# seung-lab/chunkflow

Hardware: AMD Instinct MI355X
Metric: output_voxels_per_sec (higher is better)
Workload: dtype f32; 1 GPU; config2-512cube-rsunet-affinity; batch_size=12, engine=rsunet

## Files before the change

chunkflow_amd/csrc/conv.hip:

```cpp
#include <hip/hip_runtime.h>

#include "cfx_internal.h"

namespace {

typedef float f32x4 __attribute__((ext_vector_type(4)));

constexpr int padc(int C) {
    return (C % 32 == 0 || C % 32 == 16) ? C + 4 : C;
}

template <int C, int K, int TZv, int TY, int TX, int TAPG, int NTHREADS>
__global__ __launch_bounds__(NTHREADS, 1) void k_conv3(
    const float* __restrict__ in,
    const float* __restrict__ wgt,
    const float* __restrict__ bias,
    const float* __restrict__ res,
    float* __restrict__ out,
    int N, int D, int H, int W, int do_elu) {
    constexpr int PC = padc(C);
    constexpr int SX = TX + 2;
    constexpr int SY = TY + 2;
    constexpr int SZ = TZv + 2;
    constexpr int KK = C / 4;
    constexpr int NT = (K + 15) / 16;
    constexpr int NW = NTHREADS / 64;
    constexpr int XT = TX / 16;
    constexpr int M_TILES = (TZv * TY * XT) / NW;
    static_assert((TZv * TY * XT) % NW == 0, "tiles must split evenly");

    __shared__ float slab[SZ * SY * SX * PC];
    __shared__ float wtile[TAPG * NT * C * 16];

    const int bx = blockIdx.x;
    const int by = blockIdx.y;
    const int bzn = blockIdx.z;
    const int zblocks = (D + TZv - 1) / TZv;
    const int n = bzn / zblocks;
    const int z0 = (bzn % zblocks) * TZv;
    const int y0 = by * TY;
    const int x0 = bx * TX;

    const int tid = threadIdx.x;
    const int wave = tid >> 6;
    const int lane = tid & 63;

    {
        const int c4n = C / 4;
        const int vox = SZ * SY * SX;
        const bool interior = z0 >= 1 && z0 + TZv + 1 <= D && y0 >= 1 &&
                              y0 + TY + 1 <= H && x0 >= 1 &&
                              x0 + TX + 1 <= W;
        const float* base =
            in + ((((long long)n * D + z0 - 1) * H + y0 - 1) * W + x0 - 1)
                 * C;
        if (interior) {
            for (int idx = tid; idx < vox * c4n; idx += NTHREADS) {
                const int c4 = idx % c4n;
                const int v = idx / c4n;
                const int sx = v % SX;
                const int sy = (v / SX) % SY;
                const int sz = v / (SX * SY);
                const f32x4 val = *reinterpret_cast<const f32x4*>(
                    base + (((long long)sz * H + sy) * W + sx) * C +
                    c4 * 4);
                *reinterpret_cast<f32x4*>(
                    &slab[((sz * SY + sy) * SX + sx) * PC + c4 * 4]) = val;
            }
        } else {
            for (int idx = tid; idx < vox * c4n; idx += NTHREADS) {
                const int c4 = idx % c4n;
                const int v = idx / c4n;
                const int sx = v % SX;
                const int sy = (v / SX) % SY;
                const int sz = v / (SX * SY);
                const int gz = z0 + sz - 1;
                const int gy = y0 + sy - 1;
                const int gx = x0 + sx - 1;
                const bool ok = gz >= 0 && gz < D && gy >= 0 && gy < H &&
                                gx >= 0 && gx < W;
                const int cz = ok ? gz : 0;
                const int cy = ok ? gy : 0;
                const int cx = ok ? gx : 0;
                f32x4 val = *reinterpret_cast<const f32x4*>(
                    in + ((((long long)n * D + cz) * H + cy) * W + cx) * C +
                    c4 * 4);
                if (!ok) val = {0.f, 0.f, 0.f, 0.f};
                *reinterpret_cast<f32x4*>(
                    &slab[((sz * SY + sy) * SX + sx) * PC + c4 * 4]) = val;
            }
        }
    }
    __syncthreads();

    int tmz[M_TILES], tmy[M_TILES], tmx[M_TILES];
#pragma unroll
    for (int m = 0; m < M_TILES; ++m) {
        const int g = wave * M_TILES + m;
        tmx[m] = (g % XT) * 16;
        tmy[m] = (g / XT) % TY;
        tmz[m] = g / (XT * TY);
    }

    f32x4 acc[M_TILES][NT];
#pragma unroll
    for (int m = 0; m < M_TILES; ++m)
#pragma unroll
        for (int t = 0; t < NT; ++t)
            acc[m][t] = {0.f, 0.f, 0.f, 0.f};

    const int a_row = lane & 15;
    const int a_k = lane >> 4;
    const int col16 = lane & 15;

    static_assert(27 % TAPG == 0, "TAPG must divide 27");
    for (int g = 0; g < 27 / TAPG; ++g) {
        for (int idx = tid; idx < TAPG * NT * C * 16;
             idx += NTHREADS) {
            const int j = idx & 15;
            const int c = (idx >> 4) % C;
            const int nt = (idx >> 4) / C % NT;
            const int tl = (idx >> 4) / C / NT;
            const int jg = nt * 16 + j;
            wtile[idx] = jg < K
                ? wgt[((long long)(g * TAPG + tl) * C + c) * K + jg]
                : 0.f;
        }
        __syncthreads();
#pragma unroll
        for (int tl = 0; tl < TAPG; ++tl) {
            const int tap = g * TAPG + tl;
            const int dz = tap / 9 - 1;
            const int dy = (tap / 3) % 3 - 1;
            const int dx = tap % 3 - 1;
            const float* arow[M_TILES];
#pragma unroll
            for (int m = 0; m < M_TILES; ++m) {
                arow[m] = &slab[(((1 + tmz[m] + dz) * SY +
                                  (1 + tmy[m] + dy)) * SX +
                                 (1 + tmx[m] + dx)) * PC + a_row * PC + a_k];
            }
            const float* wblk = &wtile[tl * NT * C * 16];
#pragma unroll
            for (int nt = 0; nt < NT; ++nt) {
#pragma unroll
                for (int kk = 0; kk < KK; ++kk) {
                    const float b =
                        wblk[(nt * C + kk * 4 + a_k) * 16 + col16];
#pragma unroll
                    for (int m = 0; m < M_TILES; ++m) {
                        const float a = arow[m][kk * 4];
                        acc[m][nt] = __builtin_amdgcn_mfma_f32_16x16x4f32(
                            a, b, acc[m][nt], 0, 0, 0);
                    }
                }
            }
        }
        __syncthreads();
    }

    const int col = lane & 15;
    const int rbase = (lane >> 4) * 4;
#pragma unroll
    for (int m = 0; m < M_TILES; ++m) {
        const int gz = z0 + tmz[m];
        const int gy = y0 + tmy[m];
        if (gz >= D || gy >= H) continue;
#pragma unroll
        for (int t = 0; t < NT; ++t) {
            const int j = t * 16 + col;
            if (j >= K) continue;
            const float bj = bias ? bias[j] : 0.f;
#pragma unroll
            for (int r = 0; r < 4; ++r) {
                const int gx = x0 + tmx[m] + rbase + r;
                if (gx >= W) continue;
                long long o =
                    ((((long long)n * D + gz) * H + gy) * W + gx) * K + j;
                float v = acc[m][t][r] + bj;
                if (res) v += res[o];
                if (do_elu) v = v > 0.f ? v : expm1f(v);
                out[o] = v;
            }
        }
    }
}

}

extern "C" int cfx_conv3_ndhwc(cfx_ctx* ctx, const float* in,
                               const float* wgt, const float* bias,
                               const float* residual, float* out, int N,
                               int D, int H, int W, int C, int K,
                               int do_elu) {
    if (C != K) {
        g_err = "cfx_conv3_ndhwc: only C == K widths are instantiated";
        return -1;
    }
#define CFX_CONV_CASE(CW, TZV, TYV, TXV, TAPGV, NTH)                         \
    case CW: {                                                               \
        const int zb = (D + TZV - 1) / TZV;                                  \
        dim3 grid((W + TXV - 1) / TXV, (H + TYV - 1) / TYV,                  \
                  (unsigned)(N * zb));                                       \
        hipEvent_t e0;                                                       \
        if (prof_begin(ctx, &e0)) return -1;                                 \
        hipLaunchKernelGGL((k_conv3<CW, CW, TZV, TYV, TXV, TAPGV, NTH>),     \
                           grid, dim3(NTH), 0, ctx->stream, in, wgt, bias,   \
                           residual, out, N, D, H, W, do_elu);               \
        CFX_CHECK(hipGetLastError());                                        \
        double flops = 2.0 * 27.0 * CW * CW * (double)N * D * H * W;         \
        if (prof_end(ctx, e0, CFX_K_CONV, flops)) return -1;                 \
        break;                                                               \
    }
    switch (C) {
        CFX_CONV_CASE(28, 1, 8, 32, 3, 512)
        CFX_CONV_CASE(36, 1, 8, 32, 1, 512)
        CFX_CONV_CASE(48, 1, 4, 32, 1, 512)
        CFX_CONV_CASE(64, 2, 2, 16, 1, 256)
        default:
            g_err = "cfx_conv3_ndhwc: unsupported channel width";
            return -1;
    }
#undef CFX_CONV_CASE
    return 0;
}

namespace {

template <int C, int K, int TY, int TAPG>
__global__ __launch_bounds__(512, 1) void k_conv3_w32(
    const float* __restrict__ in, const float* __restrict__ wgt,
    const float* __restrict__ bias, const float* __restrict__ res,
    float* __restrict__ out, int N, int D, int H, int W, int do_elu) {
    constexpr int TX = 32;
    constexpr int SX = TX + 2;
    constexpr int SY = TY + 2;
    constexpr int SZ = 3;
    constexpr int KK = C / 2;
    static_assert(K <= 32 && C % 2 == 0, "");

    __shared__ float slab[SZ * SY * C * SX];
    __shared__ float wtile[TAPG * C * 32];

    const int zblocks = D;
    const int n = blockIdx.z / zblocks;
    const int z0 = blockIdx.z % zblocks;
    const int y0 = blockIdx.y * TY;
    const int x0 = blockIdx.x * TX;
    const int tid = threadIdx.x;
    const int wave = tid >> 6;
    const int lane = tid & 63;

    {
        const int c4n = C / 4;
        const bool interior = z0 >= 1 && z0 + 2 <= D && y0 >= 1 &&
                              y0 + TY + 1 <= H && x0 >= 1 &&
                              x0 + TX + 1 <= W;
        for (int idx = tid; idx < SZ * SY * SX * c4n; idx += 512) {
            const int c4 = idx % c4n;
            const int v = idx / c4n;
            const int sx = v % SX;
            const int sy = (v / SX) % SY;
            const int sz = v / (SX * SY);
            const int gz = z0 + sz - 1;
            const int gy = y0 + sy - 1;
            const int gx = x0 + sx - 1;
            f32x4 val;
            if (interior) {
                val = *reinterpret_cast<const f32x4*>(
                    in + ((((long long)n * D + gz) * H + gy) * W + gx) * C +
                    c4 * 4);
            } else {
                const bool ok = gz >= 0 && gz < D && gy >= 0 && gy < H &&
                                gx >= 0 && gx < W;
                val = *reinterpret_cast<const f32x4*>(
                    in + ((((long long)n * D + (ok ? gz : 0)) * H +
                           (ok ? gy : 0)) * W + (ok ? gx : 0)) * C +
                    c4 * 4);
                if (!ok) val = {0.f, 0.f, 0.f, 0.f};
            }
            float* base = &slab[((sz * SY + sy) * C + c4 * 4) * SX + sx];
            base[0 * SX] = val.x;
            base[1 * SX] = val.y;
            base[2 * SX] = val.z;
            base[3 * SX] = val.w;
        }
    }
    __syncthreads();

    typedef float f32x16 __attribute__((ext_vector_type(16)));
    f32x16 acc = {};
    const int ax = lane & 31;
    const int ak = lane >> 5;

    static_assert(27 % TAPG == 0, "");
    for (int g = 0; g < 27 / TAPG; ++g) {
        for (int idx = tid; idx < TAPG * C * 32; idx += 512) {
            const int j = idx & 31;
            const int c = (idx >> 5) % C;
            const int tl = (idx >> 5) / C;
            wtile[idx] = j < K
                ? wgt[((long long)(g * TAPG + tl) * C + c) * K + j]
                : 0.f;
        }
        __syncthreads();
#pragma unroll
        for (int tl = 0; tl < TAPG; ++tl) {
            const int tap = g * TAPG + tl;
            const int dz = tap / 9 - 1;
            const int dy = (tap / 3) % 3 - 1;
            const int dx = tap % 3 - 1;
            const float* arow =
                &slab[((1 + dz) * SY + (1 + wave + dy)) * C * SX +
                      (1 + dx) + ax];
            const float* wrow = &wtile[tl * C * 32 + ax];
#pragma unroll
            for (int kk = 0; kk < KK; ++kk) {
                const float a = arow[(kk * 2 + ak) * SX];
                const float b = wrow[(kk * 2 + ak) * 32];
                acc = __builtin_amdgcn_mfma_f32_32x32x2f32(a, b, acc, 0, 0,
                                                           0);
            }
        }
        __syncthreads();
    }

    const int gz = z0;
    const int gy = y0 + wave;
    const int j = lane & 31;
    if (gy < H && j < K) {
        const float bj = bias ? bias[j] : 0.f;
#pragma unroll
        for (int r = 0; r < 16; ++r) {
            const int row = (r & 3) + 8 * (r >> 2) + 4 * (lane >> 5);
            const int gx = x0 + row;
            if (gx >= W) continue;
            long long o =
                ((((long long)n * D + gz) * H + gy) * W + gx) * K + j;
            float v = acc[r] + bj;
            if (res) v += res[o];
            if (do_elu) v = v > 0.f ? v : expm1f(v);
            out[o] = v;
        }
    }
}

}

extern "C" int cfx_conv3_ndhwc_w32(cfx_ctx* ctx, const float* in,
                                   const float* wgt, const float* bias,
                                   const float* residual, float* out, int N,
                                   int D, int H, int W, int C, int K,
                                   int do_elu) {
    if (C != 28 || K != 28) {
        g_err = "cfx_conv3_ndhwc_w32: only C == K == 28 instantiated";
        return -1;
    }
    dim3 grid((W + 31) / 32, (H + 7) / 8, (unsigned)(N * D));
    hipEvent_t e0;
    if (prof_begin(ctx, &e0)) return -1;
    hipLaunchKernelGGL((k_conv3_w32<28, 28, 8, 3>), grid, dim3(512), 0,
                       ctx->stream, in, wgt, bias, residual, out, N, D, H,
                       W, do_elu);
    CFX_CHECK(hipGetLastError());
    double flops = 2.0 * 27.0 * 28 * 28 * (double)N * D * H * W;
    if (prof_end(ctx, e0, CFX_K_CONV, flops)) return -1;
    return 0;
}

namespace {

template <int C, int K, int TY, int TX, int NTK>
__global__ __launch_bounds__(512, 1) void k_conv3_zring_pl(
    const float* __restrict__ in, const float* __restrict__ wgt,
    const float* __restrict__ bias, const float* __restrict__ res,
    float* __restrict__ out, int N, int D, int H, int W, int do_elu,
    int j0, int wvec) {
    constexpr int PC = padc(C);
    constexpr int SX = TX + 2;
    constexpr int SY = TY + 2;
    constexpr int KK = C / 4;
    constexpr int NT = NTK;
    constexpr int NW = 8;
    constexpr int XT = TX / 16;
    constexpr int M_TILES = (TY * XT) / NW;
    constexpr int C4N = C / 4;
    constexpr int LV = (SY * SX * C4N + 511) / 512;
    constexpr int WV4 = 27 * NT * C * 4;
    constexpr int WL = (WV4 + 511) / 512;
    static_assert((TY * XT) % NW == 0, "");

    __shared__ __attribute__((aligned(16))) float ring[3 * SY * SX * PC];
    __shared__ __attribute__((aligned(16))) float wall[27 * NT * C * 16];

    const int n = blockIdx.z;
    const int y0 = blockIdx.y * TY;
    const int x0 = blockIdx.x * TX;
    const int tid = threadIdx.x;
    const int wave = tid >> 6;
    const int lane = tid & 63;

    auto wall_load = [&](f32x4 (&wv)[WL], bool (&wk)[WL]) {
#pragma unroll
        for (int li = 0; li < WL; ++li) {
            const int idx = min(tid + li * 512, WV4 - 1);
            const int row = idx >> 2;
            const int c = row % C;
            const int nt = row / C % NT;
            const int tap = row / C / NT;
            const int jg = j0 + nt * 16 + (idx & 3) * 4;
            wk[li] = jg < K;
            wv[li] = *reinterpret_cast<const f32x4*>(
                wgt + ((long long)tap * C + c) * K + (jg < K ? jg : 0));
        }
    };
    auto wall_store = [&](const f32x4 (&wv)[WL], const bool (&wk)[WL]) {
#pragma unroll
        for (int li = 0; li < WL; ++li) {
            const int idx = tid + li * 512;
            if (idx >= WV4) break;
            *reinterpret_cast<f32x4*>(&wall[idx * 4]) =
                wk[li] ? wv[li] : f32x4{0.f, 0.f, 0.f, 0.f};
        }
    };
    if (!wvec) {
        for (int idx = tid; idx < 27 * NT * C * 16; idx += 512) {
            const int j = idx & 15;
            const int c = (idx >> 4) % C;
            const int nt = (idx >> 4) / C % NT;
            const int tap = (idx >> 4) / C / NT;
            const int jg = j0 + nt * 16 + j;
            wall[idx] =
                jg < K ? wgt[((long long)tap * C + c) * K + jg] : 0.f;
        }
    }

    const bool xy_interior = y0 >= 1 && y0 + TY + 1 <= H && x0 >= 1 &&
                             x0 + TX + 1 <= W;

    static_assert(SY * SX * C4N > 512 && SY * SX * C4N > (LV - 1) * 512, "");
    auto plane_idx = [&](int li) {
        const int idx = tid + li * 512;
        return idx < SY * SX * C4N ? idx : idx - 512;
    };
    auto plane_load = [&](int P, f32x4 (&vals)[LV], bool (&keep)[LV]) {
        const bool zin = P >= 0 && P < D;
        const bool interior = zin && xy_interior;
#pragma unroll
        for (int li = 0; li < LV; ++li) {
            const int idx = plane_idx(li);
            const int c4 = idx % C4N;
            const int v = idx / C4N;
            const int gy = y0 + v / SX - 1;
            const int gx = x0 + v % SX - 1;
            const bool ok = zin && (interior ||
                                    (gy >= 0 && gy < H && gx >= 0 &&
                                     gx < W));
            keep[li] = ok;
            vals[li] = *reinterpret_cast<const f32x4*>(
                in + ((((long long)n * D + (zin ? P : 0)) * H +
                       (ok ? gy : 0)) * W + (ok ? gx : 0)) * C + c4 * 4);
        }
    };
    auto plane_store = [&](int P, const f32x4 (&vals)[LV],
                           const bool (&keep)[LV]) {
        const int slot = ((P + 1) % 3 + 3) % 3;
#pragma unroll
        for (int li = 0; li < LV; ++li) {
            const int idx = plane_idx(li);
            const int c4 = idx % C4N;
            const int v = idx / C4N;
            *reinterpret_cast<f32x4*>(
                &ring[(slot * SY * SX + v) * PC + c4 * 4]) =
                keep[li] ? vals[li] : f32x4{0.f, 0.f, 0.f, 0.f};
        }
    };

    {
        f32x4 wv[WL];
        bool wk[WL];
        f32x4 v0[LV], v1[LV];
        bool k0[LV], k1[LV];
        if (wvec) wall_load(wv, wk);
        plane_load(-1, v0, k0);
        plane_load(0, v1, k1);
        if (wvec) wall_store(wv, wk);
        plane_store(-1, v0, k0);
        plane_store(0, v1, k1);
    }
    __syncthreads();

    int tmy[M_TILES], tmx[M_TILES];
#pragma unroll
    for (int m = 0; m < M_TILES; ++m) {
        const int g = wave * M_TILES + m;
        tmx[m] = (g % XT) * 16;
        tmy[m] = g / XT;
    }
    const int a_row = lane & 15;
    const int a_k = lane >> 4;
    const int col16 = lane & 15;
    const int colj = lane & 15;
    const int rbase = (lane >> 4) * 4;

    float bj[NT];
#pragma unroll
    for (int t = 0; t < NT; ++t)
        bj[t] = bias ? bias[min(j0 + t * 16 + colj, K - 1)] : 0.f;

    for (int z = 0; z < D; ++z) {
        f32x4 acc[M_TILES][NT];
        f32x4 acc2[M_TILES];
#pragma unroll
        for (int m = 0; m < M_TILES; ++m) {
            acc2[m] = {0.f, 0.f, 0.f, 0.f};
#pragma unroll
            for (int t = 0; t < NT; ++t)
                acc[m][t] = {0.f, 0.f, 0.f, 0.f};
        }

        auto compute_dzi = [&](int dzi) {
            const int slot = ((z + dzi) % 3 + 3) % 3;
            const float* plane = &ring[slot * SY * SX * PC];
#pragma unroll
            for (int tl = 0; tl < 9; ++tl) {
                const int tap = dzi * 9 + tl;
                const int dy = tl / 3 - 1;
                const int dx = tl % 3 - 1;
                const float* arow[M_TILES];
#pragma unroll
                for (int m = 0; m < M_TILES; ++m) {
                    arow[m] = &plane[((1 + tmy[m] + dy) * SX +
                                      (1 + tmx[m] + dx)) * PC +
                                     a_row * PC + a_k];
                }
                const float* wblk = &wall[tap * NT * C * 16];
#pragma unroll
                for (int kk = 0; kk < KK; ++kk) {
                    float a[M_TILES];
#pragma unroll
                    for (int m = 0; m < M_TILES; ++m)
                        a[m] = arow[m][kk * 4];
#pragma unroll
                    for (int nt = 0; nt < NT; ++nt) {
                        const float b =
                            wblk[(nt * C + kk * 4 + a_k) * 16 + col16];
#pragma unroll
                        for (int m = 0; m < M_TILES; ++m) {
                            f32x4& dst = (NT == 1 && (kk & 1))
                                             ? acc2[m] : acc[m][nt];
                            dst = __builtin_amdgcn_mfma_f32_16x16x4f32(
                                a[m], b, dst, 0, 0, 0);
                        }
                    }
                }
            }
        };

        f32x4 vals[LV];
        bool keep[LV];
        plane_load(z + 1, vals, keep);
        __builtin_amdgcn_sched_barrier(0);
        compute_dzi(0);
        compute_dzi(1);
        __builtin_amdgcn_sched_barrier(0);
        plane_store(z + 1, vals, keep);
        __syncthreads();

        float rv[M_TILES][NT][4];
        if (res) {
#pragma unroll
            for (int m = 0; m < M_TILES; ++m) {
                const int gym = min(y0 + tmy[m], H - 1);
#pragma unroll
                for (int t = 0; t < NT; ++t) {
                    const int jm = min(j0 + t * 16 + colj, K - 1);
#pragma unroll
                    for (int r = 0; r < 4; ++r) {
                        const int gxm = min(x0 + tmx[m] + rbase + r, W - 1);
                        rv[m][t][r] = res[
                            ((((long long)n * D + z) * H + gym) * W + gxm) *
                                K + jm];
                    }
                }
            }
        }
        compute_dzi(2);

        float ov[M_TILES][NT][4];
#pragma unroll
        for (int m = 0; m < M_TILES; ++m) {
#pragma unroll
            for (int t = 0; t < NT; ++t) {
#pragma unroll
                for (int r = 0; r < 4; ++r) {
                    float v = acc[m][t][r] + bj[t];
                    if (NT == 1) v += acc2[m][r];
                    if (res) v += rv[m][t][r];
                    if (do_elu) {
                        const float e = expm1f(v > 0.f ? 0.f : v);
                        v = v > 0.f ? v : e;
                    }
                    ov[m][t][r] = v;
                }
            }
        }
#pragma unroll
        for (int m = 0; m < M_TILES; ++m) {
            const int gy = y0 + tmy[m];
            if (gy >= H) continue;
#pragma unroll
            for (int t = 0; t < NT; ++t) {
                const int j = j0 + t * 16 + colj;
                if (j >= K) continue;
#pragma unroll
                for (int r = 0; r < 4; ++r) {
                    const int gx = x0 + tmx[m] + rbase + r;
                    if (gx >= W) continue;
                    out[((((long long)n * D + z) * H + gy) * W + gx) * K +
                        j] = ov[m][t][r];
                }
            }
        }
    }
}

template <int C, int K, int TY, int TX>
__global__ __launch_bounds__(512, 1) void k_conv3_zring_dw(
    const float* __restrict__ in, const float* __restrict__ wgt,
    const float* __restrict__ bias, const float* __restrict__ res,
    float* __restrict__ out, int N, int D, int H, int W, int do_elu,
    int j0) {
    constexpr int PC = (C % 32 == 16) ? C + 2 : padc(C);
    constexpr int SX = TX + 2;
    constexpr int SY = TY + 2;
    constexpr int KK = C / 4;
    constexpr int NW = 8;
    constexpr int XT = TX / 16;
    constexpr int M_TILES = (TY * XT) / NW;
    constexpr int C4N = C / 4;
    constexpr int LV = (SY * SX * C4N + 511) / 512;
    static_assert((TY * XT) % NW == 0, "");

    __shared__ float ring[3 * SY * SX * PC];
    __shared__ float wall[2][9 * C * 16];

    const int n = blockIdx.z;
    const int y0 = blockIdx.y * TY;
    const int x0 = blockIdx.x * TX;
    const int tid = threadIdx.x;
    const int wave = tid >> 6;
    const int lane = tid & 63;

    auto wall_store = [&](int g, int buf) {
        for (int idx = tid; idx < 9 * C * 16; idx += 512) {
            const int j = idx & 15;
            const int c = (idx >> 4) % C;
            const int tl = (idx >> 4) / C;
            const int jg = j0 + j;
            wall[buf][idx] =
                jg < K ? wgt[((long long)(9 * g + tl) * C + c) * K + jg]
                       : 0.f;
        }
    };

    const bool xy_interior = y0 >= 1 && y0 + TY + 1 <= H && x0 >= 1 &&
                             x0 + TX + 1 <= W;
    auto plane_load = [&](int P, f32x4 (&vals)[LV]) {
        const bool zin = P >= 0 && P < D;
        const bool interior = zin && xy_interior;
#pragma unroll
        for (int li = 0; li < LV; ++li) {
            const int idx = tid + li * 512;
            if (idx >= SY * SX * C4N) break;
            const int c4 = idx % C4N;
            const int v = idx / C4N;
            const int gy = y0 + v / SX - 1;
            const int gx = x0 + v % SX - 1;
            if (interior) {
                vals[li] = *reinterpret_cast<const f32x4*>(
                    in + ((((long long)n * D + P) * H + gy) * W + gx) * C +
                    c4 * 4);
            } else {
                const bool ok = zin && gy >= 0 && gy < H && gx >= 0 &&
                                gx < W;
                vals[li] = *reinterpret_cast<const f32x4*>(
                    in + ((((long long)n * D + (zin ? P : 0)) * H +
                           (ok ? gy : 0)) * W + (ok ? gx : 0)) * C +
                    c4 * 4);
                if (!ok) vals[li] = {0.f, 0.f, 0.f, 0.f};
            }
        }
    };
    typedef float f32x2 __attribute__((ext_vector_type(2)));
    auto plane_store = [&](int P, const f32x4 (&vals)[LV]) {
        const int slot = ((P + 1) % 3 + 3) % 3;
#pragma unroll
        for (int li = 0; li < LV; ++li) {
            const int idx = tid + li * 512;
            if (idx >= SY * SX * C4N) break;
            const int c4 = idx % C4N;
            const int v = idx / C4N;
            float* dst = &ring[(slot * SY * SX + v) * PC + c4 * 4];
            *reinterpret_cast<f32x2*>(dst) = f32x2{vals[li][0], vals[li][1]};
            *reinterpret_cast<f32x2*>(dst + 2) =
                f32x2{vals[li][2], vals[li][3]};
        }
    };

    {
        f32x4 v0[LV], v1[LV];
        plane_load(-1, v0);
        plane_load(0, v1);
        plane_store(-1, v0);
        plane_store(0, v1);
        wall_store(0, 0);
    }
    __syncthreads();

    int tmy[M_TILES], tmx[M_TILES];
#pragma unroll
    for (int m = 0; m < M_TILES; ++m) {
        const int g = wave * M_TILES + m;
        tmx[m] = (g % XT) * 16;
        tmy[m] = g / XT;
    }
    const int a_row = lane & 15;
    const int a_k = lane >> 4;
    const int col16 = lane & 15;
    const int colj = lane & 15;
    const int rbase = (lane >> 4) * 4;

    for (int z = 0; z < D; ++z) {
        f32x4 acc[M_TILES];
#pragma unroll
        for (int m = 0; m < M_TILES; ++m)
            acc[m] = {0.f, 0.f, 0.f, 0.f};

        auto compute_dzi = [&](int dzi, int buf) {
            const int slot = ((z + dzi) % 3 + 3) % 3;
            const float* plane = &ring[slot * SY * SX * PC];
            const float* wb = wall[buf];
#pragma unroll
            for (int tl = 0; tl < 9; ++tl) {
                const int dy = tl / 3 - 1;
                const int dx = tl % 3 - 1;
                const float* arow[M_TILES];
#pragma unroll
                for (int m = 0; m < M_TILES; ++m) {
                    arow[m] = &plane[((1 + tmy[m] + dy) * SX +
                                      (1 + tmx[m] + dx)) * PC +
                                     a_row * PC + a_k];
                }
                const float* wblk = &wb[tl * C * 16];
#pragma unroll
                for (int kk = 0; kk < KK; ++kk) {
                    const float b = wblk[(kk * 4 + a_k) * 16 + col16];
#pragma unroll
                    for (int m = 0; m < M_TILES; ++m) {
                        const float a = arow[m][kk * 4];
                        acc[m] = __builtin_amdgcn_mfma_f32_16x16x4f32(
                            a, b, acc[m], 0, 0, 0);
                    }
                }
            }
        };

        const int p = (3 * z) % 2;
        f32x4 vals[LV];
        plane_load(z + 1, vals);
        wall_store(1, 1 - p);
        compute_dzi(0, p);
        __syncthreads();
        wall_store(2, p);
        compute_dzi(1, 1 - p);
        plane_store(z + 1, vals);
        __syncthreads();
        if (z + 1 < D)
            wall_store(0, 1 - p);
        compute_dzi(2, p);

#pragma unroll
        for (int m = 0; m < M_TILES; ++m) {
            const int gy = y0 + tmy[m];
            if (gy >= H) continue;
            const int j = j0 + colj;
            if (j >= K) continue;
            const float bj = bias ? bias[j] : 0.f;
#pragma unroll
            for (int r = 0; r < 4; ++r) {
                const int gx = x0 + tmx[m] + rbase + r;
                if (gx >= W) continue;
                long long o =
                    ((((long long)n * D + z) * H + gy) * W + gx) * K + j;
                float v = acc[m][r] + bj;
                if (res) v += res[o];
                if (do_elu) v = v > 0.f ? v : expm1f(v);
                out[o] = v;
            }
        }
        __syncthreads();
    }
}

}

extern "C" int cfx_conv3_ndhwc_zring(cfx_ctx* ctx, const float* in,
                                     const float* wgt, const float* bias,
                                     const float* residual, float* out,
                                     int N, int D, int H, int W, int C,
                                     int K, int do_elu) {
    dim3 grid((W + 15) / 16, (H + 7) / 8, (unsigned)N);
    hipEvent_t e0;
    if (prof_begin(ctx, &e0)) return -1;
    const int wvec =
        (reinterpret_cast<uintptr_t>(wgt) % 16 == 0 && K % 4 == 0) ? 1 : 0;
    if (C == 28 && K == 28) {
        hipLaunchKernelGGL((k_conv3_zring_pl<28, 28, 8, 16, 2>), grid,
                           dim3(512), 0, ctx->stream, in, wgt, bias,
                           residual, out, N, D, H, W, do_elu, 0, wvec);
    } else if (C == 36 && K == 36) {
        for (int j0 = 0; j0 < 36; j0 += 16) {
            hipLaunchKernelGGL((k_conv3_zring_pl<36, 36, 8, 16, 1>), grid,
                               dim3(512), 0, ctx->stream, in, wgt, bias,
                               residual, out, N, D, H, W, do_elu, j0, wvec);
        }
    } else if (C == 48 && K == 48) {
        for (int j0 = 0; j0 < 48; j0 += 16) {
            hipLaunchKernelGGL((k_conv3_zring_dw<48, 48, 8, 16>), grid,
                               dim3(512), 0, ctx->stream, in, wgt, bias,
                               residual, out, N, D, H, W, do_elu, j0);
        }
    } else {
        g_err = "cfx_conv3_ndhwc_zring: width not instantiated";
        return -1;
    }
    CFX_CHECK(hipGetLastError());
    double flops = 2.0 * 27.0 * C * K * (double)N * D * H * W;
    if (prof_end(ctx, e0, CFX_K_CONV, flops)) return -1;
    return 0;
}

namespace {

typedef __bf16 cfx_bf16;
typedef cfx_bf16 bf16x8 __attribute__((ext_vector_type(8)));
typedef float f32x16 __attribute__((ext_vector_type(16)));

template <int C, int K, int TY, int TX>
__global__ __launch_bounds__(512, 1) void k_conv3_zring_bf16_a(
    const cfx_bf16* __restrict__ in,
    const cfx_bf16* __restrict__ wgt,
    const float* __restrict__ bias,
    const cfx_bf16* __restrict__ res,
    cfx_bf16* __restrict__ out,
    int N, int D, int H, int W, int do_elu) {
    constexpr int CP = 32;
    constexpr int PCB = CP + 8;
    constexpr int SX = TX + 2;
    constexpr int SY = TY + 2;
    constexpr int C4 = CP / 4;
    constexpr int LV = (SY * SX * C4 + 511) / 512;
    typedef cfx_bf16 bf16x4 __attribute__((ext_vector_type(4)));
    typedef cfx_bf16 bf16x8w __attribute__((ext_vector_type(8)));
    static_assert(C <= CP && K <= 32, "");

    __shared__ cfx_bf16 ring[3 * SY * SX * PCB];
    __shared__ cfx_bf16 wall[27 * 32 * PCB];
    __shared__ cfx_bf16 oscr[8][16][32];

    const int n = blockIdx.z;
    const int y0 = blockIdx.y * TY;
    const int x0 = blockIdx.x * TX;
    const int tid = threadIdx.x;
    const int wave = tid >> 6;
    const int lane = tid & 63;

    for (int idx = tid; idx < 27 * 32 * CP; idx += 512) {
        const int c = idx % CP;
        const int j = (idx / CP) % 32;
        const int tap = idx / (CP * 32);
        wall[(tap * 32 + j) * PCB + c] = wgt[(tap * 32 + j) * 32 + c];
    }

    const bool xy_interior = y0 >= 1 && y0 + TY + 1 <= H && x0 >= 1 &&
                             x0 + TX + 1 <= W;

    auto plane_load = [&](int P, bf16x4 (&vals)[LV], bool (&keep)[LV]) {
        const bool zin = P >= 0 && P < D;
        const bool interior = zin && xy_interior;
#pragma unroll
        for (int li = 0; li < LV; ++li) {
            const int idx = min(tid + li * 512, SY * SX * C4 - 1);
            const int c4 = idx % C4;
            const int v = idx / C4;
            const int gy = y0 + v / SX - 1;
            const int gx = x0 + v % SX - 1;
            const bool cok = c4 * 4 < C;
            const bool ok = cok && zin &&
                            (interior || (gy >= 0 && gy < H && gx >= 0 &&
                                          gx < W));
            keep[li] = ok;
            vals[li] = *reinterpret_cast<const bf16x4*>(
                in + ((((long long)n * D + (zin ? P : 0)) * H +
                       (ok ? gy : 0)) * W + (ok ? gx : 0)) * C +
                (cok ? c4 * 4 : 0));
        }
    };
    auto plane_store = [&](int P, const bf16x4 (&vals)[LV],
                           const bool (&keep)[LV]) {
        const int slot = ((P + 1) % 3 + 3) % 3;
#pragma unroll
        for (int li = 0; li < LV; ++li) {
            const int idx = tid + li * 512;
            if (idx >= SY * SX * C4) break;
            const int c4 = idx % C4;
            const int v = idx / C4;
            *reinterpret_cast<bf16x4*>(
                &ring[((slot * SY + v / SX) * SX + v % SX) * PCB +
                      c4 * 4]) = keep[li] ? vals[li] : bf16x4{};
        }
    };

    {
        bf16x4 v0[LV], v1[LV];
        bool k0[LV], k1[LV];
        plane_load(-1, v0, k0);
        plane_load(0, v1, k1);
        plane_store(-1, v0, k0);
        plane_store(0, v1, k1);
    }
    __syncthreads();
    bf16x4 va[LV];
    bool ka[LV];
    plane_load(1, va, ka);

    const int ax = lane & 31;
    const int khalf = (lane >> 5) * 8;

    for (int z = 0; z < D; ++z) {
        f32x16 accA = {};
        f32x16 accB = {};
        const cfx_bf16* planes[3];
#pragma unroll
        for (int dzi = 0; dzi < 3; ++dzi)
            planes[dzi] = &ring[(((z + dzi) % 3 + 3) % 3) * SY * SX * PCB];
        auto addrA = [&](int p) {
            const int tap = p >> 1, kk = p & 1;
            const int dzi = tap / 9, tl = tap % 9;
            const int dy = tl / 3 - 1, dx = tl % 3 - 1;
            return reinterpret_cast<const bf16x8*>(
                &planes[dzi][((1 + wave + dy) * SX + (1 + dx) + ax) * PCB +
                             khalf + kk * 16]);
        };
        auto addrB = [&](int p) {
            const int tap = p >> 1, kk = p & 1;
            return reinterpret_cast<const bf16x8*>(
                &wall[(tap * 32 + ax) * PCB + khalf + kk * 16]);
        };
        constexpr int PD = 4;

        bf16x4 vals[LV];
        bool keep[LV];
        plane_load(z + 2, vals, keep);
        {
            bf16x8 abuf[PD], bbuf[PD];
#pragma unroll
            for (int p = 0; p < PD; ++p) {
                abuf[p] = *addrA(p);
                bbuf[p] = *addrB(p);
            }
#pragma unroll
            for (int p = 0; p < 36; ++p) {
                const int si = p % PD;
                if (p & 1)
                    accB = __builtin_amdgcn_mfma_f32_32x32x16_bf16(
                        abuf[si], bbuf[si], accB, 0, 0, 0);
                else
                    accA = __builtin_amdgcn_mfma_f32_32x32x16_bf16(
                        abuf[si], bbuf[si], accA, 0, 0, 0);
                __builtin_amdgcn_sched_barrier(0);
                if (p + PD < 36) {
                    abuf[si] = *addrA(p + PD);
                    bbuf[si] = *addrB(p + PD);
                }
                __builtin_amdgcn_sched_barrier(0);
            }
            plane_store(z + 1, va, ka);
            __syncthreads();
#pragma unroll
            for (int p = 36; p < 36 + PD; ++p) {
                abuf[p % PD] = *addrA(p);
                bbuf[p % PD] = *addrB(p);
            }
#pragma unroll
            for (int p = 36; p < 54; ++p) {
                const int si = p % PD;
                if (p & 1)
                    accB = __builtin_amdgcn_mfma_f32_32x32x16_bf16(
                        abuf[si], bbuf[si], accB, 0, 0, 0);
                else
                    accA = __builtin_amdgcn_mfma_f32_32x32x16_bf16(
                        abuf[si], bbuf[si], accA, 0, 0, 0);
                __builtin_amdgcn_sched_barrier(0);
                if (p + PD < 54) {
                    abuf[si] = *addrA(p + PD);
                    bbuf[si] = *addrB(p + PD);
                }
                __builtin_amdgcn_sched_barrier(0);
            }
        }

#pragma unroll
        for (int li = 0; li < LV; ++li) {
            va[li] = vals[li];
            ka[li] = keep[li];
        }
        const f32x16 acc = accA + accB;
        const int gy = y0 + wave;
        const int j = lane & 31;
        const float bj = (bias && j < K) ? bias[j] : 0.f;
#pragma unroll
        for (int h = 0; h < 2; ++h) {
#pragma unroll
            for (int r = 8 * h; r < 8 * h + 8; ++r) {
                const int row = (r & 3) + 8 * ((r >> 2) & 1) +
                                4 * (lane >> 5);
                oscr[wave][row][j] = (cfx_bf16)(acc[r] + bj);
            }
            const int xr = lane >> 2;
            const int ch = lane & 3;
            const int gx = x0 + 16 * h + xr;
            if (gy < H && gx < W) {
                const int j0 = ch * 8;
                long long o = ((((long long)n * D + z) * H + gy) *
                               W + gx) * K + j0;
                if (j0 + 8 <= K) {
                    bf16x8w v = *reinterpret_cast<const bf16x8w*>(
                        &oscr[wave][xr][j0]);
#pragma unroll
                    for (int e = 0; e < 8; ++e) {
                        float t = (float)v[e];
                        if (res) t += (float)res[o + e];
                        if (do_elu) t = t > 0.f ? t : expm1f(t);
                        v[e] = (cfx_bf16)t;
                    }
                    *reinterpret_cast<bf16x8w*>(out + o) = v;
                } else if (j0 < K) {
                    bf16x4 v = *reinterpret_cast<const bf16x4*>(
                        &oscr[wave][xr][j0]);
#pragma unroll
                    for (int e = 0; e < 4; ++e) {
                        float t = (float)v[e];
                        if (res) t += (float)res[o + e];
                        if (do_elu) t = t > 0.f ? t : expm1f(t);
                        v[e] = (cfx_bf16)t;
                    }
                    *reinterpret_cast<bf16x4*>(out + o) = v;
                }
            }
        }
    }
}

template <int CPV, int TY, int TX>
__global__ __launch_bounds__(512, 1) void k_conv3_zring_bf16_s(
    const cfx_bf16* __restrict__ in, const cfx_bf16* __restrict__ wgt,
    const float* __restrict__ bias, const cfx_bf16* __restrict__ res,
    cfx_bf16* __restrict__ out, int N, int D, int H, int W, int CS,
    int CL, int c0, int KS, int Ktot, int j0, int do_elu) {
    constexpr int CP = CPV;
    constexpr int PCB = CP + 8;
    constexpr int SX = TX + 2;
    constexpr int SY = TY + 2;
    constexpr int KK = CP / 16;
    constexpr int C4 = CP / 4;
    constexpr int LV = (SY * SX * C4 + 511) / 512;
    typedef cfx_bf16 bf16x4 __attribute__((ext_vector_type(4)));
    constexpr int WPK = 64;
    constexpr int WPC = 48;

    __shared__ cfx_bf16 ring[3 * SY * SX * PCB];
    __shared__ cfx_bf16 wall[27 * 32 * PCB];
    __shared__ cfx_bf16 oscr[8][16][32];

    const int n = blockIdx.z;
    const int y0 = blockIdx.y * TY;
    const int x0 = blockIdx.x * TX;
    const int tid = threadIdx.x;
    const int wave = tid >> 6;
    const int lane = tid & 63;

    for (int idx = tid; idx < 27 * 32 * CP; idx += 512) {
        const int c = idx % CP;
        const int j = (idx / CP) % 32;
        const int tap = idx / (CP * 32);
        wall[(tap * 32 + j) * PCB + c] =
            wgt[(tap * WPK + j0 + j) * WPC + c0 + c];
    }

    const bool xy_interior = y0 >= 1 && y0 + TY + 1 <= H && x0 >= 1 &&
                             x0 + TX + 1 <= W;

    auto plane_load = [&](int P, bf16x4 (&vals)[LV], bool (&keep)[LV]) {
        const bool zin = P >= 0 && P < D;
        const bool interior = zin && xy_interior;
#pragma unroll
        for (int li = 0; li < LV; ++li) {
            const int idx = min(tid + li * 512, SY * SX * C4 - 1);
            const int c4 = idx % C4;
            const int v = idx / C4;
            const int gy = y0 + v / SX - 1;
            const int gx = x0 + v % SX - 1;
            const bool cok = c4 * 4 < CL;
            const bool ok = cok && zin &&
                            (interior || (gy >= 0 && gy < H && gx >= 0 &&
                                          gx < W));
            keep[li] = ok;
            vals[li] = *reinterpret_cast<const bf16x4*>(
                in + (((long long)n * D + (zin ? P : 0)) * H +
                      (ok ? gy : 0)) * (long long)W * CS +
                (ok ? gx : 0) * (long long)CS + c0 + (cok ? c4 * 4 : 0));
        }
    };
    auto plane_store = [&](int P, const bf16x4 (&vals)[LV],
                           const bool (&keep)[LV]) {
        const int slot = ((P + 1) % 3 + 3) % 3;
#pragma unroll
        for (int li = 0; li < LV; ++li) {
            const int idx = tid + li * 512;
            if (idx >= SY * SX * C4) break;
            const int c4 = idx % C4;
            const int v = idx / C4;
            *reinterpret_cast<bf16x4*>(
                &ring[((slot * SY + v / SX) * SX + v % SX) * PCB +
                      c4 * 4]) = keep[li] ? vals[li] : bf16x4{};
        }
    };

    {
        bf16x4 v0[LV], v1[LV];
        bool k0[LV], k1[LV];
        plane_load(-1, v0, k0);
        plane_load(0, v1, k1);
        plane_store(-1, v0, k0);
        plane_store(0, v1, k1);
    }
    __syncthreads();

    const int ax = lane & 31;
    const int khalf = (lane >> 5) * 8;

    for (int z = 0; z < D; ++z) {
        f32x16 acc = {};
        f32x16 accB = {};
        const cfx_bf16* planes[3];
#pragma unroll
        for (int dzi = 0; dzi < 3; ++dzi)
            planes[dzi] = &ring[(((z + dzi) % 3 + 3) % 3) * SY * SX * PCB];
        auto addrA = [&](int p) {
            const int tap = p / KK, kk = p % KK;
            const int dzi = tap / 9, tl = tap % 9;
            const int dy = tl / 3 - 1, dx = tl % 3 - 1;
            return reinterpret_cast<const bf16x8*>(
                &planes[dzi][((1 + wave + dy) * SX + (1 + dx) + ax) * PCB +
                             khalf + kk * 16]);
        };
        auto addrB = [&](int p) {
            const int tap = p / KK, kk = p % KK;
            return reinterpret_cast<const bf16x8*>(
                &wall[(tap * 32 + ax) * PCB + khalf + kk * 16]);
        };
        constexpr int PD = 4;
        constexpr int NP1 = 18 * KK;
        constexpr int NP2 = 27 * KK;

        bf16x4 vals[LV];
        bool keep[LV];
        plane_load(z + 1, vals, keep);
        {
            bf16x8 abuf[PD], bbuf[PD];
#pragma unroll
            for (int p = 0; p < PD; ++p) {
                abuf[p] = *addrA(p);
                bbuf[p] = *addrB(p);
            }
#pragma unroll
            for (int p = 0; p < NP1; ++p) {
                const int si = p % PD;
                if (p & 1)
                    accB = __builtin_amdgcn_mfma_f32_32x32x16_bf16(
                        abuf[si], bbuf[si], accB, 0, 0, 0);
                else
                    acc = __builtin_amdgcn_mfma_f32_32x32x16_bf16(
                        abuf[si], bbuf[si], acc, 0, 0, 0);
                __builtin_amdgcn_sched_barrier(0);
                if (p + PD < NP1) {
                    abuf[si] = *addrA(p + PD);
                    bbuf[si] = *addrB(p + PD);
                }
                __builtin_amdgcn_sched_barrier(0);
            }
            plane_store(z + 1, vals, keep);
            __syncthreads();
#pragma unroll
            for (int p = NP1; p < NP1 + PD; ++p) {
                abuf[p % PD] = *addrA(p);
                bbuf[p % PD] = *addrB(p);
            }
#pragma unroll
            for (int p = NP1; p < NP2; ++p) {
                const int si = p % PD;
                if (p & 1)
                    accB = __builtin_amdgcn_mfma_f32_32x32x16_bf16(
                        abuf[si], bbuf[si], accB, 0, 0, 0);
                else
                    acc = __builtin_amdgcn_mfma_f32_32x32x16_bf16(
                        abuf[si], bbuf[si], acc, 0, 0, 0);
                __builtin_amdgcn_sched_barrier(0);
                if (p + PD < NP2) {
                    abuf[si] = *addrA(p + PD);
                    bbuf[si] = *addrB(p + PD);
                }
                __builtin_amdgcn_sched_barrier(0);
            }
        }

        acc = acc + accB;
        const int gy = y0 + wave;
        const int j = lane & 31;
        if (gy < H) {
            const float bj =
                (bias && j0 + j < Ktot) ? bias[j0 + j] : 0.f;
#pragma unroll
            for (int h = 0; h < 2; ++h) {
#pragma unroll
                for (int r = 8 * h; r < 8 * h + 8; ++r) {
                    const int row = (r & 3) + 8 * ((r >> 2) & 1) +
                                    4 * (lane >> 5);
                    oscr[wave][row][j] = (cfx_bf16)(acc[r] + bj);
                }
                const int xr = lane >> 2;
                const int ch = lane & 3;
                const int gx = x0 + 16 * h + xr;
                const int rem = Ktot - j0 - ch * 8;
                if (gx < W && rem >= 4) {
                    const int j0c = ch * 8;
                    long long o = (((long long)n * D + z) * H + gy) *
                                      (long long)W * KS +
                                  (long long)gx * KS + j0 + j0c;
                    typedef cfx_bf16 bf16x8s
                        __attribute__((ext_vector_type(8)));
                    if (rem >= 8) {
                        bf16x8s v = *reinterpret_cast<const bf16x8s*>(
                            &oscr[wave][xr][j0c]);
#pragma unroll
                        for (int e = 0; e < 8; ++e) {
                            float t = (float)v[e];
                            if (res) t += (float)res[o + e];
                            if (do_elu) t = t > 0.f ? t : expm1f(t);
                            v[e] = (cfx_bf16)t;
                        }
                        *reinterpret_cast<bf16x8s*>(out + o) = v;
                    } else {
                        bf16x4 v = *reinterpret_cast<const bf16x4*>(
                            &oscr[wave][xr][j0c]);
#pragma unroll
                        for (int e = 0; e < 4; ++e) {
                            float t = (float)v[e];
                            if (res) t += (float)res[o + e];
                            if (do_elu) t = t > 0.f ? t : expm1f(t);
                            v[e] = (cfx_bf16)t;
                        }
                        *reinterpret_cast<bf16x4*>(out + o) = v;
                    }
                }
            }
        }
    }
}

}

extern "C" int cfx_conv3_ndhwc_bf16(cfx_ctx* ctx, const void* in,
                                    const void* wgt, const float* bias,
                                    const void* residual, void* out, int N,
                                    int D, int H, int W, int C, int K,
                                    int do_elu) {
    if ((C == 36 && K == 36) || (C == 48 && K == 48)) {
        dim3 grid((W + 31) / 32, (H + 7) / 8, (unsigned)N);
        hipEvent_t e0;
        if (prof_begin(ctx, &e0)) return -1;
        const int CL2 = C - 32;
        for (int j0 = 0; j0 < K; j0 += 32) {
            hipLaunchKernelGGL((k_conv3_zring_bf16_s<32, 8, 32>), grid,
                               dim3(512), 0, ctx->stream,
                               (const cfx_bf16*)in, (const cfx_bf16*)wgt,
                               nullptr, (const cfx_bf16*)residual,
                               (cfx_bf16*)out, N, D, H, W, C, 32, 0, K, K,
                               j0, 0);
            hipLaunchKernelGGL((k_conv3_zring_bf16_s<16, 8, 32>), grid,
                               dim3(512), 0, ctx->stream,
                               (const cfx_bf16*)in, (const cfx_bf16*)wgt,
                               bias, (const cfx_bf16*)out, (cfx_bf16*)out,
                               N, D, H, W, C, CL2, 32, K, K, j0, do_elu);
        }
        CFX_CHECK(hipGetLastError());
        double flops = 2.0 * 27.0 * C * K * (double)N * D * H * W;
        if (prof_end(ctx, e0, CFX_K_CONV, flops)) return -1;
        return 0;
    }
    if (C != 28 || K != 28) {
        g_err = "cfx_conv3_ndhwc_bf16: only C == K == 28/36/48 instantiated";
        return -1;
    }
    dim3 grid((W + 31) / 32, (H + 7) / 8, (unsigned)N);
    hipEvent_t e0;
    if (prof_begin(ctx, &e0)) return -1;
    hipLaunchKernelGGL((k_conv3_zring_bf16_a<28, 28, 8, 32>), grid,
                       dim3(512), 0, ctx->stream, (const cfx_bf16*)in,
                       (const cfx_bf16*)wgt, bias, (const cfx_bf16*)residual,
                       (cfx_bf16*)out, N, D, H, W, do_elu);
    CFX_CHECK(hipGetLastError());
    double flops = 2.0 * 27.0 * 28 * 28 * (double)N * D * H * W;
    if (prof_end(ctx, e0, CFX_K_CONV, flops)) return -1;
    return 0;
}
```

Baseline: 110.4 million voxels/s.

## Fold 36-channel remainder columns into first pass using 4x4x1 MFMA

For the C=K=36 conv, the third pass over output channels 32..35 previously ran a full 16-wide MFMA tile, mostly padding. Those 4 channels are now computed inside the first pass with 4x4x1 MFMA instructions plus cross-lane shuffle reductions, cutting the launches from three to two. This avoids re-reading the input planes and wasting three quarters of a tile on zero columns. In exchange the first pass needs more shared memory for weights, more registers and more instructions, and the 4x4 MFMA path may have lower throughput.

```diff
diff --git a/chunkflow_amd/csrc/conv.hip b/chunkflow_amd/csrc/conv.hip
--- a/chunkflow_amd/csrc/conv.hip
+++ b/chunkflow_amd/csrc/conv.hip
@@ -370,7 +370,7 @@
 
 namespace {
 
-template <int C, int K, int TY, int TX, int NTK>
+template <int C, int K, int TY, int TX, int NTK, int NT4, int J4>
 __global__ __launch_bounds__(512, 1) void k_conv3_zring_pl(
     const float* __restrict__ in, const float* __restrict__ wgt,
     const float* __restrict__ bias, const float* __restrict__ res,
@@ -381,17 +381,22 @@
     constexpr int SY = TY + 2;
     constexpr int KK = C / 4;
     constexpr int NT = NTK;
+    constexpr int N4 = NT4 > 0 ? NT4 : 1;
     constexpr int NW = 8;
     constexpr int XT = TX / 16;
     constexpr int M_TILES = (TY * XT) / NW;
     constexpr int C4N = C / 4;
     constexpr int LV = (SY * SX * C4N + 511) / 512;
-    constexpr int WV4 = 27 * NT * C * 4;
+    constexpr int W16 = 27 * NT * C * 16;
+    constexpr int W16V4 = W16 / 4;
+    constexpr int WV4 = W16V4 + 27 * NT4 * C;
     constexpr int WL = (WV4 + 511) / 512;
+    constexpr bool SPLIT = NT == 1;
     static_assert((TY * XT) % NW == 0, "");
+    static_assert(NT4 == 0 || (J4 % 4 == 0 && J4 + 4 * NT4 <= K), "");
 
     __shared__ __attribute__((aligned(16))) float ring[3 * SY * SX * PC];
-    __shared__ __attribute__((aligned(16))) float wall[27 * NT * C * 16];
+    __shared__ __attribute__((aligned(16))) float wall[WV4 * 4];
 
     const int n = blockIdx.z;
     const int y0 = blockIdx.y * TY;
@@ -404,11 +409,12 @@
 #pragma unroll
         for (int li = 0; li < WL; ++li) {
             const int idx = min(tid + li * 512, WV4 - 1);
-            const int row = idx >> 2;
+            const bool blk = NT4 > 0 && idx >= W16V4;
+            const int row = blk ? idx - W16V4 : idx >> 2;
             const int c = row % C;
-            const int nt = row / C % NT;
-            const int tap = row / C / NT;
-            const int jg = j0 + nt * 16 + (idx & 3) * 4;
+            const int nt = blk ? row / C % N4 : row / C % NT;
+            const int tap = blk ? row / C / N4 : row / C / NT;
+            const int jg = blk ? J4 + nt * 4 : j0 + nt * 16 + (idx & 3) * 4;
             wk[li] = jg < K;
             wv[li] = *reinterpret_cast<const f32x4*>(
                 wgt + ((long long)tap * C + c) * K + (jg < K ? jg : 0));
@@ -424,7 +430,7 @@
         }
     };
     if (!wvec) {
-        for (int idx = tid; idx < 27 * NT * C * 16; idx += 512) {
+        for (int idx = tid; idx < W16; idx += 512) {
             const int j = idx & 15;
             const int c = (idx >> 4) % C;
             const int nt = (idx >> 4) / C % NT;
@@ -432,6 +438,13 @@
             const int jg = j0 + nt * 16 + j;
             wall[idx] =
                 jg < K ? wgt[((long long)tap * C + c) * K + jg] : 0.f;
+        }
+        for (int idx = tid; idx < 27 * NT4 * C * 4; idx += 512) {
+            const int c = (idx >> 2) % C;
+            const int t = (idx >> 2) / C % N4;
+            const int tap = (idx >> 2) / C / N4;
+            wall[W16 + idx] = wgt[((long long)tap * C + c) * K + J4 +
+                                  t * 4 + (idx & 3)];
         }
     }
 
@@ -507,16 +520,28 @@
 #pragma unroll
     for (int t = 0; t < NT; ++t)
         bj[t] = bias ? bias[min(j0 + t * 16 + colj, K - 1)] : 0.f;
+    const int col4 = lane & 3;
+    const int pos4 = ((lane >> 2) & 3) * 4 + (lane >> 4);
+    float bj4[N4];
+#pragma unroll
+    for (int t = 0; t < NT4; ++t)
+        bj4[t] = bias ? bias[J4 + t * 4 + col4] : 0.f;
+    int w4lane = W16 + a_k * 4 + col4;
+    asm volatile("" : "+v"(w4lane));
 
     for (int z = 0; z < D; ++z) {
         f32x4 acc[M_TILES][NT];
         f32x4 acc2[M_TILES];
+        f32x4 acc4[M_TILES][N4];
 #pragma unroll
         for (int m = 0; m < M_TILES; ++m) {
             acc2[m] = {0.f, 0.f, 0.f, 0.f};
 #pragma unroll
             for (int t = 0; t < NT; ++t)
                 acc[m][t] = {0.f, 0.f, 0.f, 0.f};
+#pragma unroll
+            for (int t = 0; t < N4; ++t)
+                acc4[m][t] = {0.f, 0.f, 0.f, 0.f};
         }
 
         auto compute_dzi = [&](int dzi) {
@@ -535,6 +560,7 @@
                                      a_row * PC + a_k];
                 }
                 const float* wblk = &wall[tap * NT * C * 16];
+                const float* wblk4 = &wall[w4lane + tap * NT4 * C * 4];
 #pragma unroll
                 for (int kk = 0; kk < KK; ++kk) {
                     float a[M_TILES];
@@ -547,12 +573,22 @@
                             wblk[(nt * C + kk * 4 + a_k) * 16 + col16];
 #pragma unroll
                         for (int m = 0; m < M_TILES; ++m) {
-                            f32x4& dst = (NT == 1 && (kk & 1))
+                            f32x4& dst = (SPLIT && (kk & 1))
                                              ? acc2[m] : acc[m][nt];
                             dst = __builtin_amdgcn_mfma_f32_16x16x4f32(
                                 a[m], b, dst, 0, 0, 0);
                         }
                     }
+#pragma unroll
+                    for (int t = 0; t < NT4; ++t) {
+                        const float b4 =
+                            wblk4[(t * C + kk * 4) * 4];
+#pragma unroll
+                        for (int m = 0; m < M_TILES; ++m)
+                            acc4[m][t] = __builtin_amdgcn_mfma_f32_4x4x1f32(
+                                a[m], b4, acc4[m][t], 0, 0, 0);
+                    }
+                    if (NT4 > 0) __builtin_amdgcn_sched_barrier(0x106);
                 }
             }
         };
@@ -568,10 +604,17 @@
         __syncthreads();
 
         float rv[M_TILES][NT][4];
+        float rv4[M_TILES][N4];
         if (res) {
 #pragma unroll
             for (int m = 0; m < M_TILES; ++m) {
                 const int gym = min(y0 + tmy[m], H - 1);
+                const int gx4 = min(x0 + tmx[m] + pos4, W - 1);
+#pragma unroll
+                for (int t = 0; t < NT4; ++t)
+                    rv4[m][t] = res[
+                        ((((long long)n * D + z) * H + gym) * W + gx4) * K +
+                        J4 + t * 4 + col4];
 #pragma unroll
                 for (int t = 0; t < NT; ++t) {
                     const int jm = min(j0 + t * 16 + colj, K - 1);
@@ -605,10 +648,39 @@
                 }
             }
         }
+        float ov4[M_TILES][N4];
+#pragma unroll
+        for (int m = 0; m < M_TILES; ++m) {
+#pragma unroll
+            for (int t = 0; t < NT4; ++t) {
+                float v = 0.f;
+#pragma unroll
+                for (int i = 0; i < 4; ++i) {
+                    float s = acc4[m][t][i];
+                    s += __shfl_xor(s, 32);
+                    s += __shfl_xor(s, 16);
+                    v = a_k == i ? s : v;
+                }
+                v += bj4[t];
+                if (res) v += rv4[m][t];
+                if (do_elu) {
+                    const float e = expm1f(v > 0.f ? 0.f : v);
+                    v = v > 0.f ? v : e;
+                }
+                ov4[m][t] = v;
+            }
+        }
 #pragma unroll
         for (int m = 0; m < M_TILES; ++m) {
             const int gy = y0 + tmy[m];
             if (gy >= H) continue;
+            const int gx4 = x0 + tmx[m] + pos4;
+#pragma unroll
+            for (int t = 0; t < NT4; ++t) {
+                if (gx4 >= W) continue;
+                out[((((long long)n * D + z) * H + gy) * W + gx4) * K + J4 +
+                    t * 4 + col4] = ov4[m][t];
+            }
 #pragma unroll
             for (int t = 0; t < NT; ++t) {
                 const int j = j0 + t * 16 + colj;
@@ -816,15 +888,16 @@
     const int wvec =
         (reinterpret_cast<uintptr_t>(wgt) % 16 == 0 && K % 4 == 0) ? 1 : 0;
     if (C == 28 && K == 28) {
-        hipLaunchKernelGGL((k_conv3_zring_pl<28, 28, 8, 16, 2>), grid,
-                           dim3(512), 0, ctx->stream, in, wgt, bias,
+        hipLaunchKernelGGL((k_conv3_zring_pl<28, 28, 8, 16, 2, 0, 0>),
+                           grid, dim3(512), 0, ctx->stream, in, wgt, bias,
                            residual, out, N, D, H, W, do_elu, 0, wvec);
     } else if (C == 36 && K == 36) {
-        for (int j0 = 0; j0 < 36; j0 += 16) {
-            hipLaunchKernelGGL((k_conv3_zring_pl<36, 36, 8, 16, 1>), grid,
-                               dim3(512), 0, ctx->stream, in, wgt, bias,
-                               residual, out, N, D, H, W, do_elu, j0, wvec);
-        }
+        hipLaunchKernelGGL((k_conv3_zring_pl<36, 36, 8, 16, 1, 1, 32>),
+                           grid, dim3(512), 0, ctx->stream, in, wgt, bias,
+                           residual, out, N, D, H, W, do_elu, 0, wvec);
+        hipLaunchKernelGGL((k_conv3_zring_pl<36, 36, 8, 16, 1, 0, 0>),
+                           grid, dim3(512), 0, ctx->stream, in, wgt, bias,
+                           residual, out, N, D, H, W, do_elu, 16, wvec);
     } else if (C == 48 && K == 48) {
         for (int j0 = 0; j0 < 48; j0 += 16) {
             hipLaunchKernelGGL((k_conv3_zring_dw<48, 48, 8, 16>), grid,
```

Measured after the change: 117.4 million voxels/s, median of 6. 6.3% higher.
